# ssilverman16/particle_col_image_segmentation

Hardware: AMD Instinct MI355X
Metric: Mpixels/sec segmented (5-ch 1024x1024 TIFF), ROI mask IoU=1.0 (higher is better)
Workload: dtype f32 planes / u8 class maps / int32 labels / f64 ROI sums; 1 GPU; BASELINE config 2: batch of 64 frames 1024x1024x5 float32 per GPU, full kernel chain, inputs resident in HBM; frames_per_gpu=64, height=1024, width=1024, planes=5, parallelism=frames x1, launch=one hipGraph replay per step, 4 in flight, tie_fallback_frames_last_step=0, reference_nan_frames_rank0=0

## Files before the change

### particle_col_image_segmentation_amd/csrc/ccl.hip

```cpp
#include <type_traits>

#include "column_pass.h"
#include "tile_ops.h"

namespace pcseg {

constexpr int SCAN_PIX = 1024;

struct KeyEqU8 {
    const uint8_t *p;
    int W;
    int64_t n;
    __device__ __forceinline__ int operator()(int b, int r, int c) const { return p[b * n + rowoff(r, W) + c]; }
};
struct KeyNzU8 {
    const uint8_t *p;
    int W;
    int64_t n;
    __device__ __forceinline__ int operator()(int b, int r, int c) const { return p[b * n + rowoff(r, W) + c] != 0; }
};
struct KeyZeroU8 {
    const uint8_t *p;
    int W;
    int64_t n;
// ... 620 lines not shown
    if (ch == 0) u0 = u1l = u1r = 0;
    if (ch + 1 >= nch) d0 = d1l = d1r = 0;
    const unsigned cur1 = w0 | w1l | w1r, prev1 = u0 | u1l | u1r, next1 = d0 | d1l | d1r;
    unsigned acc = cur1 | w2l | w2r;
    acc |= (cur1 << 1) | (prev1 >> 31) | (cur1 >> 1) | (next1 << 31);
    acc |= (w0 << 2) | (u0 >> 30) | (w0 >> 2) | (d0 << 30);
    const int rows = min(32, H - ch * 32);
    acc &= col_valid(rows);
    out[((int64_t)b * nch + ch) * W + c] = acc;
}

constexpr int BR_TW = 64, BR_CH = 4, BR_ROWS = 32 * BR_CH;

__device__ __forceinline__ int bitrun_start(unsigned word, int p)
{
    const unsigned below = ~word & ((1u << p) - 1u);
    return below ? 32 - __clz(below) : 0;
}

template <typename Link>
__device__ __forceinline__ void bitrun_left_links(unsigned w, unsigned wl, Link &&link)
{
    unsigned rest = wl ? w : 0u;
    while (rest) {
        const int a = __ffs(rest) - 1;
        const unsigned from_a = w >> a;
        const int len = from_a == 0xFFFFFFFFu ? 32 : __ffs(~from_a) - 1;
        const int e = a + len - 1;
        rest = e >= 31 ? 0u : rest & ~((2u << e) - 1u);
        const int lo = max(a - 1, 0), hi = min(e + 1, 31);
        unsigned m = wl & (hi == 31 ? 0xFFFFFFFFu : ((2u << hi) - 1u)) & ~((1u << lo) - 1u);
        while (m) {
            const int p = __ffs(m) - 1;
            const int st = bitrun_start(wl, p);
            const unsigned from_p = wl >> p;
            const int run_len = from_p == 0xFFFFFFFFu ? 32 : __ffs(~from_p) - 1;
            const int en = p + run_len - 1;
            m = en >= 31 ? 0u : m & ~((2u << en) - 1u);
            link(a, st);
        }
    }
}

__global__ void __launch_bounds__(256) bitrun_tile_kernel(const unsigned *__restrict__ bits, int *__restrict__ parent, int H, int W,
                                                           int nch)
{
    __shared__ unsigned sw[BR_CH][BR_TW];
    __shared__ int lpar[BR_ROWS * BR_TW];
    const int col = threadIdx.x & (BR_TW - 1), q = threadIdx.x >> 6;
    const int c0 = blockIdx.x * BR_TW, ch0 = blockIdx.y * BR_CH, b = blockIdx.z;
    const int c = c0 + col, ch = ch0 + q;
    const unsigned w = (c < W && ch < nch) ? bits[((int64_t)b * nch + ch) * W + c] : 0u;
    sw[q][col] = w;
    for (unsigned heads = w & ~(w << 1); heads; heads &= heads - 1) {
        const int node = (q * 32 + (__ffs(heads) - 1)) * BR_TW + col;
        lpar[node] = node;
    }
    __syncthreads();
    if (w) {
        if (col > 0)
            bitrun_left_links(w, sw[q][col - 1], [&](int a, int st) {
                unite_lds(lpar, (q * 32 + a) * BR_TW + col, (q * 32 + st) * BR_TW + col - 1);
            });
        if ((w & 1u) && q > 0) {
            const int node = (q * 32) * BR_TW + col;
            const unsigned wu = sw[q - 1][col];
            if (wu >> 31) {
                unite_lds(lpar, node, ((q - 1) * 32 + bitrun_start(wu, 31)) * BR_TW + col);
            } else {
                if (col > 0 && (sw[q - 1][col - 1] >> 31))
                    unite_lds(lpar, node, ((q - 1) * 32 + bitrun_start(sw[q - 1][col - 1], 31)) * BR_TW + col - 1);
                if (col + 1 < BR_TW && (sw[q - 1][col + 1] >> 31))
                    unite_lds(lpar, node, ((q - 1) * 32 + bitrun_start(sw[q - 1][col + 1], 31)) * BR_TW + col + 1);
            }
        }
    }
    __syncthreads();
    int *par = parent + (int64_t)b * H * W;
    for (unsigned heads = w & ~(w << 1); heads; heads &= heads - 1) {
        const int node = (q * 32 + (__ffs(heads) - 1)) * BR_TW + col;
        const int root = find_lds(lpar, node);
        par[(ch0 * 32 + node / BR_TW) * W + c0 + node % BR_TW] = (ch0 * 32 + root / BR_TW) * W + c0 + root % BR_TW;
    }
}

__global__ void __launch_bounds__(256) bitrun_border_kernel(const unsigned *__restrict__ bits, int *__restrict__ parent, int H, int W,
                                                             int nch)
{
    const int c = blockIdx.x * 256 + threadIdx.x;
    const int ch = blockIdx.y, b = blockIdx.z;
    if (c >= W) return;
    const int col = c & (BR_TW - 1);
    const bool tile_left = col == 0 && c > 0, tile_top = (ch % BR_CH) == 0 && ch > 0;
    const bool edge_col = col == 0 || col == BR_TW - 1;
    if (!tile_left && !tile_top && !(edge_col && ch > 0)) return;
    const unsigned *wb = bits + (int64_t)b * nch * W;
    const int cl = c > 0 ? c - 1 : c, cr = c + 1 < W ? c + 1 : c, chu = ch > 0 ? ch - 1 : ch;
    const unsigned w = wb[rowoff(ch, W) + c], wl = wb[rowoff(ch, W) + cl];
    const unsigned wu = wb[rowoff(chu, W) + c], wul = wb[rowoff(chu, W) + cl], wur = wb[rowoff(chu, W) + cr];
    if (w == 0) return;
    int *par = parent + (int64_t)b * H * W;
    const int row0 = ch * 32;
    if (tile_left)
        bitrun_left_links(w, wl, [&](int a, int st) { unite_glb(par, (row0 + a) * W + c, (row0 + st) * W + c - 1); });
    if ((w & 1u) && ch > 0) {
        const int node = row0 * W + c;
        if (wu >> 31) {
            if (tile_top) unite_glb(par, node, (row0 - 32 + bitrun_start(wu, 31)) * W + c);
        } else {
            if (c > 0 && (tile_top || col == 0) && (wul >> 31)) unite_glb(par, node, (row0 - 32 + bitrun_start(wul, 31)) * W + c - 1);
            if (c + 1 < W && (tile_top || col == BR_TW - 1) && (wur >> 31))
                unite_glb(par, node, (row0 - 32 + bitrun_start(wur, 31)) * W + c + 1);
        }
    }
}

__global__ void __launch_bounds__(256) border_flag_kernel(const int *__restrict__ parent, uint8_t *__restrict__ flag, int H, int W)
{
    int t = blockIdx.x * blockDim.x + threadIdx.x;
    int r, c;
    if (t < W) { r = 0; c = t; }
    else if (t < 2 * W) { r = H - 1; c = t - W; }
    else if (t < 2 * W + H) { r = t - 2 * W; c = 0; }
    else if (t < 2 * W + 2 * H) { r = t - 2 * W - H; c = W - 1; }
    else return;
    int64_t fbase = (int64_t)blockIdx.y * H * W;
    int p = parent[fbase + rowoff(r, W) + c];
    if (p >= 0) flag[fbase + p] = 1;
}

__global__ void __launch_bounds__(256) fill_holes_out_kernel(const uint8_t *__restrict__ mask, const int *__restrict__ parent,
                                                              const uint8_t *__restrict__ flag, uint8_t *__restrict__ out, int64_t n)
{
    int64_t i = (int64_t)blockIdx.x * blockDim.x + threadIdx.x;
    if (i >= n) return;
    int64_t fbase = (int64_t)blockIdx.y * n;
    int p = parent[fbase + i];
    out[fbase + i] = (mask[fbase + i] != 0) || (p >= 0 && flag[fbase + p] == 0);
}

__global__ void __launch_bounds__(256) ccl_flatten_kernel(int *__restrict__ parent, int64_t n)
{
    int64_t i = (int64_t)blockIdx.x * blockDim.x + threadIdx.x;
    if (i >= n) return;
    int *par = parent + (int64_t)blockIdx.y * n;
    int p = par[i];
    if (p < 0 || !walk_ok((int)i, p)) return;
    const int x = walk_root(par, p);
    if (x != p) par[i] = x;
}

constexpr int LM_TW = CCL_TW, LM_TH = CCL_TH, LM_SW = LM_TW + 4, LM_SH = LM_TH + 4, LM_CW = LM_TW + 2, LM_CH = LM_TH + 2;

__global__ void __launch_bounds__(256) locmax_candidates_kernel(const int *__restrict__ img, unsigned long long *__restrict__ cbits,
                                                                 uint8_t *__restrict__ bad, int *__restrict__ nonconst,
                                                                 int *__restrict__ parent, int *__restrict__ markers, int H, int W)
{
    __shared__ int tile[LM_SH * LM_SW];
    __shared__ uint8_t cand[LM_CH * LM_CW];
    __shared__ int key[CCL_TILE];
    static_assert(LM_SH * LM_SW >= CCL_TILE, "the parents reuse the value tile");
    int *par = tile;
    const int OUTSIDE = (int)0x80000000;
    const TileIndex ti = xcd_tile_index();
    const int r0 = ti.y * LM_TH, c0 = ti.x * LM_TW;
    const int64_t fbase = (int64_t)ti.z * H * W;
    if ((W & 3) == 0 && c0 + LM_TW <= W && (((uintptr_t)img) & 15) == 0) {
        constexpr int QUADS = LM_SH * (LM_TW / 4), TRIPS = (QUADS + 255) / 256;
        int4 tq[TRIPS];
#pragma unroll
        for (int t = 0; t < TRIPS; ++t) {
            const int i = min((int)threadIdx.x + 256 * t, QUADS - 1);
            const int r = r0 + i / (LM_TW / 4) - 2;
            tq[t] = *reinterpret_cast<const int4 *>(img + fbase + rowoff(min(max(r, 0), H - 1), W) + c0 + 4 * (i % (LM_TW / 4)));
        }
        const int hl = min((int)threadIdx.x, LM_SH * 4 - 1);
        const int hr = r0 + (hl >> 2) - 2, hx = (hl & 3) < 2 ? (hl & 3) - 2 : LM_TW + (hl & 3) - 2, hc = c0 + hx;
        const int hv = img[fbase + rowoff(min(max(hr, 0), H - 1), W) + min(max(hc, 0), W - 1)];
#pragma unroll
        for (int t = 0; t < TRIPS; ++t) {
            const int i = (int)threadIdx.x + 256 * t;
            if (i < QUADS) {
                const int lr = i / (LM_TW / 4), r = r0 + lr - 2;
                const bool in = r >= 0 && r < H;
                int *dst = tile + lr * LM_SW + 2 + 4 * (i % (LM_TW / 4));
                dst[0] = in ? tq[t].x : OUTSIDE; dst[1] = in ? tq[t].y : OUTSIDE; dst[2] = in ? tq[t].z : OUTSIDE; dst[3] = in ? tq[t].w : OUTSIDE;
            }
        }
        if (threadIdx.x < LM_SH * 4) tile[(hl >> 2) * LM_SW + hx + 2] = (hr >= 0 && hr < H && hc >= 0 && hc < W) ? hv : OUTSIDE;
    } else {
        constexpr int TRIPS = (LM_SH * LM_SW + 255) / 256;
        int tv[TRIPS];
#pragma unroll
        for (int t = 0; t < TRIPS; ++t) {
            const int i = min((int)threadIdx.x + 256 * t, LM_SH * LM_SW - 1);
            const int r = r0 + i / LM_SW - 2, c = c0 + i % LM_SW - 2;
            tv[t] = img[fbase + rowoff(min(max(r, 0), H - 1), W) + min(max(c, 0), W - 1)];
        }
#pragma unroll
        for (int t = 0; t < TRIPS; ++t) {
            const int i = (int)threadIdx.x + 256 * t;
            const int r = r0 + i / LM_SW - 2, c = c0 + i % LM_SW - 2;
            if (i < LM_SH * LM_SW) tile[i] = (r >= 0 && r < H && c >= 0 && c < W) ? tv[t] : OUTSIDE;
        }
    }
    __syncthreads();
    const int first_value = img[fbase];
    bool any_differs = false;
    for (int t = threadIdx.x; t < LM_CH * LM_CW; t += 256) {
        const int lr = t / LM_CW, lc = t % LM_CW;
        const int r = r0 + lr - 1, c = c0 + lc - 1;
        const int i = (lr + 1) * LM_SW + lc + 1;
        const int v = tile[i];
        uint8_t state = 2;
        if (r >= 0 && r < H && c >= 0 && c < W) {
            const int *up = tile + i - LM_SW, *dn = tile + i + LM_SW;
            const int m = max(max(max(up[-1], up[0]), max(up[1], tile[i - 1])), max(max(tile[i + 1], dn[-1]), max(dn[0], dn[1])));
            state = m < v ? 1 : (m == v ? 3 : 0);
            any_differs = any_differs || v != first_value;
        }
        cand[t] = state;
    }
    __syncthreads();
    unsigned links = 0;
#pragma unroll
    for (int kk = 0; kk < LM_TH * LM_TW / 256; ++kk) {
        const int t = threadIdx.x + 256 * kk;
        const int lr = t / LM_TW, lc = t % LM_TW;
        const int r = r0 + lr, c = c0 + lc;
        int k = 0;
        if (r < H && c < W) {
            const int i = (lr + 2) * LM_SW + lc + 2, j = (lr + 1) * LM_CW + lc + 1;
            const int v = tile[i];
            const uint8_t st = cand[j];
            const bool is_cand = (st & 1) != 0;
            bool touches = false;
            if (st == 3) {
#pragma unroll
                for (int dr = -1; dr <= 1; ++dr)
#pragma unroll
                    for (int dc = -1; dc <= 1; ++dc) {
                        if (dr == 0 && dc == 0) continue;
                        const bool eq = tile[i + dr * LM_SW + dc] == v;
                        const uint8_t sn = cand[j + dr * LM_CW + dc];
                        touches = touches || (eq && sn == 0);
                        if ((dr < 0 || (dr == 0 && dc < 0)) && eq && (sn & 1) && lr + dr >= 0 && lc + dc >= 0 && lc + dc < LM_TW)
                            links |= 1u << (4 * kk + (dr == 0 ? 0 : dc + 2));
                    }
            }
            k = is_cand ? (v == 0 ? (int)0x80000000 : v) : 0;
            if (is_cand) bad[fbase + rowoff(r, W) + c] = touches ? 1 : 0;
            else if (markers) markers[fbase + rowoff(r, W) + c] = 0;
        }
        key[t] = k;
        const unsigned long long rowbits = __ballot(k != 0);
        if (lane_id() == 0 && r < H && rowbits) {
            const int64_t g = fbase + rowoff(r, W) + c0;
            const int sh = (int)(g & 63);
            atomicOr(cbits + (g >> 6), rowbits << sh);
            if (sh) atomicOr(cbits + (g >> 6) + 1, rowbits >> (64 - sh));
        }
    }
    if (__any(any_differs) && lane_id() == 0 && nonconst[ti.z] == 0) nonconst[ti.z] = 1;
    __syncthreads();
    for (int i = threadIdx.x; i < CCL_TILE; i += 256) par[i] = i;
    __syncthreads();
    if (links) {
#pragma unroll
        for (int kk = 0; kk < LM_TH * LM_TW / 256; ++kk) {
            const unsigned m = (links >> (4 * kk)) & 15u;
            if (!m) continue;
            const int i = threadIdx.x + 256 * kk;
            if (m & 1u) unite_lds_pair(par, i, i - 1);
            if (m & 2u) unite_lds_pair(par, i, i - CCL_TW - 1);
            if (m & 4u) unite_lds_pair(par, i, i - CCL_TW);
            if (m & 8u) unite_lds_pair(par, i, i - CCL_TW + 1);
        }
    }
    __syncthreads();
    for (int i = threadIdx.x; i < CCL_TILE; i += 256) {
        const int r = r0 + i / CCL_TW, c = c0 + i % CCL_TW;
        if (r >= H || c >= W || key[i] == 0) continue;
        const int root = find_lds(par, i);
        parent[fbase + rowoff(r, W) + c] = (r0 + root / CCL_TW) * W + c0 + root % CCL_TW;
    }
}

__global__ void __launch_bounds__(256) locmax_propagate_kernel(int *__restrict__ parent, uint8_t *bad,
                                                                const unsigned long long *__restrict__ cbits, int64_t n, int64_t total)
{
    const int64_t w = (int64_t)blockIdx.x * blockDim.x + threadIdx.x;
    if (w * 64 >= total) return;
    for (unsigned long long m = cbits[w]; m; m &= m - 1) {
        const int64_t g = w * 64 + (__ffsll((long long)m) - 1);
        const int64_t fbase = (g / n) * n;
        const int i = (int)(g - fbase);
        int *par = parent + fbase;
        const int p = par[i];
        if (!walk_ok(i, p)) continue;
        const int x = walk_root(par, p);
        if (x != p) par[i] = x;
        if (x != i && bad[g]) bad[fbase + x] = 1;
    }
}

__global__ void __launch_bounds__(256) locmax_out_kernel(const int *__restrict__ parent, const uint8_t *__restrict__ bad,
                                                          const int *__restrict__ nonconst, const unsigned long long *__restrict__ cbits,
                                                          uint8_t *__restrict__ is_max, int64_t n)
{
    int64_t i = (int64_t)blockIdx.x * blockDim.x + threadIdx.x;
    if (i >= n) return;
    const int64_t fbase = (int64_t)blockIdx.y * n;
    uint8_t v = 0;
    if (cand_bit(cbits, fbase + i)) v = bad[fbase + parent[fbase + i]] == 0 && nonconst[blockIdx.y] != 0;
    is_max[fbase + i] = v;
}

__device__ __forceinline__ unsigned long long cand_word(const unsigned long long *cbits, int b, int64_t i0, int64_t n)
{
    if (i0 >= n) return 0ull;
    const int64_t g0 = (int64_t)b * n + i0;
    const int sh = (int)(g0 & 63);
    unsigned long long w = cbits[g0 >> 6] >> sh;
    if (sh) w |= cbits[(g0 >> 6) + 1] << (64 - sh);
    if (n - i0 < 64) w &= (1ull << (n - i0)) - 1ull;
    return w;
}

static_assert(SCAN_PIX == 1024, "sixteen 64-bit words per count block");
template <typename Pred>
__global__ void __launch_bounds__(256) locmax_count_kernel(const int *__restrict__ parent, int *__restrict__ labels,
                                                            int *__restrict__ blockcount, const unsigned long long *__restrict__ cbits,
                                                            Pred pred, int64_t n, int nblk)
{
    const int b = blockIdx.y;
    const int *par = parent + (int64_t)b * n;
    const int64_t word = (int64_t)blockIdx.x * 256 + threadIdx.x;
    const int64_t i0 = word * 64;
    unsigned long long roots = 0;
    for (unsigned long long m = cand_word(cbits, b, i0, n); m; m &= m - 1) {
        const int j = __ffsll((long long)m) - 1;
        const int64_t i = i0 + j;
// ... 336 lines not shown
```

### particle_col_image_segmentation_amd/csrc/watershed.hip

```cpp
#include <algorithm>
#include <atomic>
#include <climits>
#include <mutex>
#include <type_traits>

#include "common.h"
#include "tile_rounds.h"

namespace pcseg {

constexpr int WS_T = 64;
constexpr unsigned WS_INF = 0xFFFFFFFFu;
constexpr int WS_CNT0 = 32, WS_CNT_STRIDE = 32, WS_CHANGED_INTS = WS_CNT0 + 16 * WS_CNT_STRIDE;

__device__ __forceinline__ unsigned ws_key(float f)
{
    if (f == 0.0f) f = 0.0f;
    unsigned u = __float_as_uint(f);
    u = (u & 0x80000000u) ? ~u : (u | 0x80000000u);
    return u == WS_INF ? WS_INF - 1 : u;
}

__global__ void __launch_bounds__(256) ws_init_kernel(const float *__restrict__ img, int64_t frame_stride,
                                                       const int *__restrict__ markers, const uint8_t *__restrict__ mask,
// ... 270 lines not shown
            if (oy >= 0 && oy < nxt.ny && ox >= 0 && ox < nxt.nx)
                mark_tile(dirty_out, list_out, count_out, ((int64_t)b * nxt.ny + oy) * nxt.nx + ox);
        }
    }
    __syncthreads();
    if (in.vec) {
#pragma unroll
        for (int t = 0; t < T * QW / NT; ++t) {
            const int idx = tid + NT * t, lr = idx / QW, q = idx % QW;
            const int r = r0 + lr, c = c0 + 4 * q;
            const uint2 *src = sLV + (lr + 1) * P + 1 + 4 * q;
            if (r >= 0 && r < H && c >= 0 && c < W)
                *reinterpret_cast<uint4 *>(L + fbase + rowoff(r, W) + c) = make_uint4(src[0].x, src[1].x, src[2].x, src[3].x);
        }
        return;
    }
    for (int i = tid; i < T * T; i += NT) {
        int lr = i / T, lc = i % T;
        int r = r0 + lr, c = c0 + lc;
        if (r >= 0 && r < H && c >= 0 && c < W) L[fbase + rowoff(r, W) + c] = sLV[(lr + 1) * P + lc + 1].x;
    }
}

__global__ void __launch_bounds__(RelaxGeom::THREADS) ws_relax_kernel(WsInputs in, const bool FIRST, unsigned *__restrict__ val,
                                                                         unsigned *__restrict__ L, uint8_t *__restrict__ dirty_in,
                                                                         uint8_t *__restrict__ dirty_out, int *__restrict__ any_changed,
                                                                         int H, int W, Tiling cur, Tiling nxt, int max_iter,
                                                                         int *__restrict__ list_out, int *__restrict__ count_out)
{
    extern __shared__ __attribute__((aligned(16))) uint2 relax_lds[];
    const TileIndex t = xcd_tile_index();
    ws_relax_tile(relax_lds + RelaxGeom::PAD, in, FIRST, val, L, dirty_in, dirty_out, any_changed, H, W, cur, nxt, max_iter, t.x, t.y,
                     t.z, list_out, count_out);
}

constexpr int WS_LIST_FROM = 4, WS_LIST_GRID = 1024;

__global__ void __launch_bounds__(RelaxGeom::THREADS) ws_relax_list_kernel(WsInputs in, unsigned *__restrict__ val, unsigned *__restrict__ L,
                                                                           uint8_t *__restrict__ dirty_in, uint8_t *__restrict__ dirty_out,
                                                                           int *__restrict__ any_changed, int H, int W, Tiling cur,
                                                                           Tiling nxt, int max_iter, TileList tiles,
                                                                           int *__restrict__ list_out, int *__restrict__ count_out)
{
    extern __shared__ __attribute__((aligned(16))) uint2 relax_lds[];
    for_tiles(tiles, [&](const int b, const int tx, const int ty) {
        ws_relax_tile(relax_lds + RelaxGeom::PAD, in, false, val, L, dirty_in, dirty_out, any_changed, H, W, cur, nxt, max_iter, tx, ty, b,
                      list_out, count_out);
        __syncthreads();
    });
}

__global__ void __launch_bounds__(RelaxGeom::THREADS) ws_relax_tail_kernel(WsInputs in, unsigned *__restrict__ val, unsigned *__restrict__ L,
                                                                           uint8_t *__restrict__ dirtyA, uint8_t *__restrict__ dirtyB,
                                                                           int *__restrict__ any_changed, int *__restrict__ not_converged,
                                                                           int *__restrict__ exact_flags, int H, int W, Tiling t0,
                                                                           Tiling t1, int first_round, int max_rounds)
{
    extern __shared__ __attribute__((aligned(16))) uint2 relax_lds[];
    const int b = blockIdx.x;
    const int rounds = tail_rounds<RelaxGeom::THREADS>(
        b, dirtyA, dirtyB, first_round, max_rounds, t0, t1, [](const int) { return true; },
        [&](const Tiling &cur, const Tiling &nxt, const int tx, const int ty, uint8_t *din, uint8_t *dout) {
            ws_relax_tile(relax_lds + RelaxGeom::PAD, in, false, val, L, din, dout, any_changed, H, W, cur, nxt, 100000, tx, ty, b);
        });
    if (rounds < 0 && threadIdx.x == 0) { *not_converged = 1; exact_flags[b] = 1; }
}

__device__ __forceinline__ bool ws_active(const uint8_t *active, int b, int r, int c, int tilesX, int tilesY)
{
    return active == nullptr || active[((int64_t)b * tilesY + r / WS_T) * tilesX + c / WS_T] != 0;
}

__global__ void __launch_bounds__(256) ws_list_tiles_kernel(const int *__restrict__ frame_list, const uint8_t *__restrict__ active, int ntpf,
                                                             int *__restrict__ tile_list)
{
    ws_for_frames(frame_list, blockIdx.x, gridDim.x, [&](const int b) {
        for (int t = threadIdx.x; t < ntpf; t += 256)
            if (active[(int64_t)b * ntpf + t]) tile_list[atomicAdd(&tile_list[-1], 1)] = b * ntpf + t;
    });
}

constexpr int UF_TW = 64, UF_TH = 32, UF_SW = UF_TW + 2, UF_SH = UF_TH + 2;
constexpr int UF_LNS = UF_TW * UF_TH;
constexpr int UF_NS = 1 << 30;

__device__ __forceinline__ int vfind_lds(int *par, int v)
{
    int p;
    while ((p = ld_lds(par + (v & (UF_LNS - 1)))) != v) {
        const int g = ld_lds(par + (p & (UF_LNS - 1)));
        if (g != p) st_lds(par + (v & (UF_LNS - 1)), g);
        v = g;
    }
    return v;
}
__device__ __forceinline__ void vunite_lds(int *par, int a, int b)
{
    for (;;) {
        a = vfind_lds(par, a);
        b = vfind_lds(par, b);
        if (a == b) return;
        if (a < b) { int t = a; a = b; b = t; }
        int old = atomicMin(&par[a & (UF_LNS - 1)], b);
        if (old == a) return;
        a = old;
    }
}
__device__ __forceinline__ bool vwalk_ok(int x, int p, int n) { return (unsigned)p <= (unsigned)x && (p & (UF_NS - 1)) < n; }

__device__ __forceinline__ void vunite_glb(int *par, int p, int q, int n, int *corrupt)
{
    int a = ld_agent(par + p), b = ld_agent(par + q);
    bool ok = a >= 0 && b >= 0 && (a & (UF_NS - 1)) < n && (b & (UF_NS - 1)) < n;
    while (ok) {
        for (;;) {
            if (a == b) return;
            const int pa = ld_agent(par + (a & (UF_NS - 1))), pb = ld_agent(par + (b & (UF_NS - 1)));
            if (pa == a && pb == b) break;
            if (!vwalk_ok(a, pa, n) || !vwalk_ok(b, pb, n)) { ok = false; break; }
            const int ga = ld_agent(par + (pa & (UF_NS - 1))), gb = ld_agent(par + (pb & (UF_NS - 1)));
            if (!vwalk_ok(pa, ga, n) || !vwalk_ok(pb, gb, n)) { ok = false; break; }
            if (pa != a) {
                if (ga != pa) __hip_atomic_store(par + (a & (UF_NS - 1)), ga, __ATOMIC_RELAXED, __HIP_MEMORY_SCOPE_AGENT);
                a = ga;
            }
            if (pb != b) {
                if (gb != pb) __hip_atomic_store(par + (b & (UF_NS - 1)), gb, __ATOMIC_RELAXED, __HIP_MEMORY_SCOPE_AGENT);
                b = gb;
            }
        }
        if (!ok) break;
        if (a == b) return;
        if (a < b) { int t = a; a = b; b = t; }
        int old = atomicMin(par + (a & (UF_NS - 1)), b);
        if (old == a) return;
        if (!vwalk_ok(a, old, n)) break;
        a = old;
    }
    walk_corrupt(corrupt);
}
__device__ __forceinline__ int vwalk_root(const int *par, int x, int n, bool &bad)
{
    int q;
    while ((q = par[x & (UF_NS - 1)]) != x) {
        if (!vwalk_ok(x, q, n)) {
            bad = true;
            break;
        }
        x = q;
    }
    return x;
}

template <typename KeyT>
__device__ __forceinline__ void ws_uf_tile_frame(KeyT *sK, int *par, uint8_t *sM, const int b, const int tile_x, const int tile_y,
                                                 const KeyT *__restrict__ K,
                                                 const int *__restrict__ F, const uint8_t *__restrict__ active,
                                                 int *__restrict__ parent, uint8_t *__restrict__ minmask, uint8_t *__restrict__ bad,
                                                 int H, int W, int tilesX, int tilesY)
{
    const KeyT KINF = ~(KeyT)0;
    const int r0 = tile_y * UF_TH, c0 = tile_x * UF_TW;
    if (!ws_active(active, b, r0, c0, tilesX, tilesY)) return;
    const int64_t fbase = (int64_t)b * H * W;
    if (sizeof(KeyT) == 4 && (W & 3) == 0 && c0 + UF_TW <= W && (((uintptr_t)K) & 15) == 0) {
        constexpr int QUADS = UF_SH * (UF_TW / 4), TRIPS = (QUADS + 255) / 256;
        uint4 kq[TRIPS];
#pragma unroll
        for (int t = 0; t < TRIPS; ++t) {
            const int i = min((int)threadIdx.x + 256 * t, QUADS - 1);
            const int r = r0 + i / (UF_TW / 4) - 1;
            kq[t] = *reinterpret_cast<const uint4 *>(K + fbase + rowoff(min(max(r, 0), H - 1), W) + c0 + 4 * (i % (UF_TW / 4)));
        }
        const int hl = min((int)threadIdx.x, UF_SH * 2 - 1);
        const int hr = r0 + (hl >> 1) - 1, hx = (hl & 1) ? UF_TW : -1, hc = c0 + hx;
        const KeyT hv = K[fbase + rowoff(min(max(hr, 0), H - 1), W) + min(max(hc, 0), W - 1)];
#pragma unroll
        for (int t = 0; t < TRIPS; ++t) {
            const int i = (int)threadIdx.x + 256 * t;
            if (i < QUADS) {
                const int lr = i / (UF_TW / 4), r = r0 + lr - 1;
                const bool in = r >= 0 && r < H;
                KeyT *dst = sK + lr * UF_SW + 1 + 4 * (i % (UF_TW / 4));
                dst[0] = in ? (KeyT)kq[t].x : KINF; dst[1] = in ? (KeyT)kq[t].y : KINF;
                dst[2] = in ? (KeyT)kq[t].z : KINF; dst[3] = in ? (KeyT)kq[t].w : KINF;
            }
        }
        if (threadIdx.x < UF_SH * 2) sK[(hl >> 1) * UF_SW + hx + 1] = (hr >= 0 && hr < H && hc >= 0 && hc < W) ? hv : KINF;
    } else {
        constexpr int TRIPS = (UF_SH * UF_SW + 255) / 256;
        KeyT kv[TRIPS];
#pragma unroll
        for (int t = 0; t < TRIPS; ++t) {
            const int i = min((int)threadIdx.x + 256 * t, UF_SH * UF_SW - 1);
            const int r = r0 + i / UF_SW - 1, c = c0 + i % UF_SW - 1;
            kv[t] = K[fbase + rowoff(min(max(r, 0), H - 1), W) + min(max(c, 0), W - 1)];
        }
#pragma unroll
        for (int t = 0; t < TRIPS; ++t) {
            const int i = (int)threadIdx.x + 256 * t;
            const int r = r0 + i / UF_SW - 1, c = c0 + i % UF_SW - 1;
            if (i < UF_SH * UF_SW) sK[i] = (r >= 0 && r < H && c >= 0 && c < W) ? kv[t] : KINF;
        }
    }
    __syncthreads();
    int self[UF_LNS / 256];
    int fv[UF_LNS / 256];
#pragma unroll
    for (int k = 0; k < UF_LNS / 256; ++k) {
        const int t = threadIdx.x + k * 256;
        fv[k] = F[fbase + rowoff(min(r0 + t / UF_TW, H - 1), W) + min(c0 + t % UF_TW, W - 1)];
    }
#pragma unroll
    for (int k = 0; k < UF_LNS / 256; ++k) {
        const int t = threadIdx.x + k * 256;
        const int lr = t / UF_TW, lc = t % UF_TW;
        const int r = r0 + lr, c = c0 + lc;
        const int i = (lr + 1) * UF_SW + lc + 1;
        int v = -1;
        if ((unsigned)(sK[i] >> (8 * sizeof(KeyT) - 32)) != WS_INF)
            v = fv[k] != 0 ? t : t + UF_LNS;
        uint8_t m8 = 0;
        if (v >= UF_LNS) {
            const KeyT ku = sK[i - UF_SW], kl = sK[i - 1], kr = sK[i + 1], kd = sK[i + UF_SW];
            const KeyT m = min(min(ku, kd), min(kl, kr));
            if (m != KINF) m8 = (ku == m ? 1 : 0) | (kl == m ? 2 : 0) | (kr == m ? 4 : 0) | (kd == m ? 8 : 0);
        }
        self[k] = v;
        sM[t] = m8;
        if (r < H && c < W) {
            minmask[fbase + rowoff(r, W) + c] = m8;
            if (fv[k] != 0) bad[fbase + rowoff(r, W) + c] = 0;
        }
    }
    __syncthreads();
#pragma unroll
    for (int k = 0; k < UF_LNS / 256; ++k) {
        const int t = threadIdx.x + k * 256;
        const int lc = t % UF_TW;
        const bool joins_left = lc > 0 && ((sM[t] & 2) || (sM[t - 1] & 4));
        const unsigned long long heads = __ballot(!joins_left);
        const unsigned long long seeds = __ballot(self[k] >= 0 && self[k] < UF_LNS);
        const unsigned long long upto = heads & (lc == 63 ? ~0ull : ((2ull << lc) - 1ull));
        const int start = 63 - __clzll((long long)upto);
        const unsigned long long later = lc == 63 ? 0ull : (heads >> (lc + 1));
        const int end = later ? lc + (__ffsll((long long)later) - 1) : 63;
        const unsigned long long run = (end == 63 ? ~0ull : ((2ull << end) - 1ull)) & ~((1ull << start) - 1ull);
        const unsigned long long run_seeds = seeds & run;
        int root = -1;
        if (self[k] >= 0) {
            if (run_seeds) root = (t - lc) + (__ffsll((long long)run_seeds) - 1);
            else root = (t - lc) + start + UF_LNS;
        }
        par[t] = root;
    }
    __syncthreads();
#pragma unroll
    for (int k = 0; k < UF_LNS / 256; ++k) {
        const int t = threadIdx.x + k * 256;
        const int lr = t / UF_TW, lc = t % UF_TW;
        if (lr == 0 || self[k] < 0) continue;
        const uint8_t m = sM[t], mu = sM[t - UF_TW];
        if (!((m & 1) || (mu & 8))) continue;
        if (lc > 0) {
            const uint8_t ml = sM[t - 1], mul = sM[t - UF_TW - 1];
            const bool same_run = (m & 2) || (ml & 4), same_run_up = (mu & 2) || (mul & 4), left_vertical = (ml & 1) || (mul & 8);
            if (same_run && same_run_up && left_vertical) continue;
        }
        vunite_lds(par, par[t], par[t - UF_TW]);
    }
    __syncthreads();
    for (int t = threadIdx.x; t < UF_TH * UF_TW; t += 256) {
        const int r = r0 + t / UF_TW, c = c0 + t % UF_TW;
        if (r >= H || c >= W) continue;
        int v = -1;
        if (par[t] >= 0) {
            const int root = vfind_lds(par, par[t]);
            const int lt = root & (UF_LNS - 1);
            v = ((r0 + lt / UF_TW) * W + c0 + lt % UF_TW) | (root >= UF_LNS ? UF_NS : 0);
        }
        parent[fbase + rowoff(r, W) + c] = v;
    }
}

template <typename KeyT, bool LIST>
__global__ void __launch_bounds__(256) ws_uf_tile_kernel(TileList tiles, const KeyT *__restrict__ K, const int *__restrict__ F,
                                                          const uint8_t *__restrict__ active, int *__restrict__ parent,
                                                          uint8_t *__restrict__ minmask, uint8_t *__restrict__ bad, int H, int W,
                                                          int tilesX, int tilesY)
{
    __shared__ KeyT sK[UF_SH * UF_SW];
    __shared__ int par[UF_TH * UF_TW];
    __shared__ uint8_t sM[UF_LNS];
    if constexpr (!LIST) {
        const TileIndex t = xcd_tile_index();
        ws_uf_tile_frame<KeyT>(sK, par, sM, t.z, t.x, t.y, K, F, active, parent, minmask, bad, H, W, tilesX, tilesY);
    } else {
        for_tiles(tiles, [&](const int b, const int tx, const int ty) {
            for (int half = 0; half < WS_T / UF_TH; ++half) {
                if ((ty * (WS_T / UF_TH) + half) * UF_TH < H)
                    ws_uf_tile_frame<KeyT>(sK, par, sM, b, tx, ty * (WS_T / UF_TH) + half, K, F, active, parent, minmask, bad, H, W, tilesX,
                                           tilesY);
                __syncthreads();
            }
        });
    }
}

__global__ void __launch_bounds__(256, 8) ws_uf_border_kernel(const int *__restrict__ frame_list, const uint8_t *__restrict__ minmask, const uint8_t *__restrict__ active,
                                                            int *__restrict__ parent, int H, int W, int tilesX, int tilesY,
                                                            int *__restrict__ exact_flags)
{
    const int n_top_rows = (H - 1) / UF_TH, n_edges = (W - 1) / UF_TW;
    int i = blockIdx.x * 256 + threadIdx.x;
    int r, c;
    if (i < n_top_rows * W) {
        r = (i / W + 1) * UF_TH;
        c = i % W;
    } else {
        i -= n_top_rows * W;
        if (i >= n_edges * H) return;
        r = i % H;
        if ((r % UF_TH) == 0 && r > 0) return;
        c = (i / H + 1) * UF_TW;
    }
    ws_for_frames(frame_list, blockIdx.y, gridDim.y, [&](const int b) {
    if (!ws_active(active, b, r, c, tilesX, tilesY)) return;
    const bool top = (r % UF_TH) == 0 && r > 0;
    const bool left = (c % UF_TW) == 0 && c > 0;
    if (!top && !left) return;
    const int64_t fbase = (int64_t)b * H * W;
    int *par = parent + fbase;
    const int p = r * W + c;
    const uint8_t *mm = minmask + fbase;
    const int up = r > 0 ? W : 0, lf = c > 0 ? 1 : 0;
    const uint8_t mp = mm[p], mu = mm[p - up], ml = mm[p - lf], mul = mm[p - up - lf];
    if (top && ws_active(active, b, r - 1, c, tilesX, tilesY)) {
        if ((mp & 1) || (mu & 8)) {
            bool implied = false;
            if (!left && c > 0) implied = ((mp & 2) || (ml & 4)) && ((mu & 2) || (mul & 4)) && ((ml & 1) || (mul & 8));
            if (!implied) vunite_glb(par, p, p - W, H * W, exact_flags + b);
        }
    }
    if (left && ws_active(active, b, r, c - 1, tilesX, tilesY)) {
        if ((mp & 2) || (ml & 4)) {
            bool implied = false;
            if (!top && r > 0) implied = ((mp & 1) || (mu & 8)) && ((ml & 1) || (mul & 8)) && ((mu & 2) || (mul & 4));
            if (!implied) vunite_glb(par, p, p - 1, H * W, exact_flags + b);
        }
    }
    });
}

enum { UF_OPTIMISTIC = 0, UF_REPAIR = 1, UF_DETECT = 2, UF_ASSIGN = 3 };

template <int MODE>
__device__ __forceinline__ void ws_uf_label_pixel(const int b, const int64_t i, const int *__restrict__ parent, int *__restrict__ F,
                                                  const uint8_t *__restrict__ active, uint8_t *__restrict__ bad,
                                                  const int *__restrict__ markers, const uint8_t *__restrict__ mask,
                                                  int *__restrict__ tie_flags, uint8_t *__restrict__ mark_active, int64_t n, int W,
                                                  int tilesX, int tilesY, int *__restrict__ exact_flags, uint8_t *__restrict__ in_bad,
                                                  uint8_t *__restrict__ mark_dirty)
{
    const int r = (int)(i / W), c = (int)(i % W);
    if (i >= n || !ws_active(active, b, r, c, tilesX, tilesY)) return;
    const int64_t fbase = (int64_t)b * n, g = fbase + i;
    if (MODE == UF_REPAIR && in_bad) in_bad[g] = 0;
    int x = parent[g];
    if (x < 0) return;
    const int *par = parent + fbase;
    bool broken = (x & (UF_NS - 1)) >= (int)n;
    if (!broken) x = vwalk_root(par, x, (int)n, broken);
    if (broken) {
        exact_flags[b] = 1;
        return;
    }
    if (x >= UF_NS) return;
    const int64_t groot = fbase + x;
    if (MODE == UF_REPAIR) {
        if (bad[groot]) {
            F[g] = mask[g] ? markers[g] : 0;
            if (mark_active) mark_active[((int64_t)b * tilesY + r / WS_T) * tilesX + c / WS_T] = 1;
            if (mark_dirty) mark_dirty[((int64_t)b * tilesY + r / WS_T) * tilesX + c / WS_T] = 1;
            if (in_bad) in_bad[g] = 1;
        }
        return;
    }
    const int f = F[g];
    if (MODE == UF_ASSIGN) {
        if (f == 0 && !bad[groot]) F[g] = F[groot];
        return;
    }
    const int lab = F[groot];
    if (f == 0) {
        if (MODE == UF_OPTIMISTIC) F[g] = lab;
    } else if (f != lab) {
        bad[groot] = 1;
        if (tie_flags[b] == 0) tie_flags[b] = 1;
    }
}

template <int MODE>
__global__ void __launch_bounds__(256) ws_uf_label_kernel(const int *__restrict__ frame_list, const int *__restrict__ parent, int *__restrict__ F,
                                                           const uint8_t *__restrict__ active, uint8_t *__restrict__ bad,
                                                           const int *__restrict__ markers, const uint8_t *__restrict__ mask,
                                                           int *__restrict__ tie_flags, uint8_t *__restrict__ mark_active, int64_t n,
                                                           int W, int tilesX, int tilesY, int *__restrict__ exact_flags,
                                                           uint8_t *__restrict__ in_bad = nullptr, uint8_t *__restrict__ mark_dirty = nullptr)
{
    const int64_t i = (int64_t)blockIdx.x * blockDim.x + threadIdx.x;
    ws_for_frames(frame_list, blockIdx.y, gridDim.y, [&](const int b) {
        ws_uf_label_pixel<MODE>(b, i, parent, F, active, bad, markers, mask, tie_flags, mark_active, n, W, tilesX, tilesY, exact_flags,
                                in_bad, mark_dirty);
    });
}

template <int MODE>
__global__ void __launch_bounds__(256) ws_uf_label_tiles_kernel(TileList tiles, const int *__restrict__ parent, int *__restrict__ F,
                                                                 const uint8_t *__restrict__ active, uint8_t *__restrict__ bad,
                                                                 const int *__restrict__ markers, const uint8_t *__restrict__ mask,
                                                                 int *__restrict__ tie_flags, int H, int W, int tilesX, int tilesY,
                                                                 int *__restrict__ exact_flags)
{
    for_tiles(tiles, [&](const int b, const int tx, const int ty) {
        ws_for_tile_pixels(tx, ty, H, W, [&](const int r, const int c) {
            ws_uf_label_pixel<MODE>(b, (int64_t)r * W + c, parent, F, active, bad, markers, mask, tie_flags, nullptr, (int64_t)H * W, W,
                                    tilesX, tilesY, exact_flags, nullptr, nullptr);
        });
    });
}

constexpr int LABEL4_Q = 3;

template <int NCH>
__device__ __forceinline__ void label4_chains(const int *par, const int *F, int64_t fbase, int n, int (&root)[NCH], int (&lab)[NCH], bool &bad)
{
    const int n1 = n - 1;
    int cut = 0;
    bool more = true;
    while (more) {
        int nx[NCH];
#pragma unroll
        for (int q = 0; q < NCH; ++q) {
            const unsigned px = (unsigned)(root[q] & (INT_MIN | (UF_NS - 1)));
            nx[q] = px <= (unsigned)n1 ? par[min(px, (unsigned)n1)] : -1;
        }
// ... 987 lines not shown
```

Baseline: 17550 Mpixels/s.

## Add wave-ballot row pass for watershed UF tile and quad-vectorized locmax candidates

```diff
diff --git a/particle_col_image_segmentation_amd/csrc/ccl.hip b/particle_col_image_segmentation_amd/csrc/ccl.hip
--- a/particle_col_image_segmentation_amd/csrc/ccl.hip
+++ b/particle_col_image_segmentation_amd/csrc/ccl.hip
@@ -796,12 +796,142 @@
 
 constexpr int LM_TW = CCL_TW, LM_TH = CCL_TH, LM_SW = LM_TW + 4, LM_SH = LM_TH + 4, LM_CW = LM_TW + 2, LM_CH = LM_TH + 2;
 
+constexpr int LM_CP = 72;
+__device__ __forceinline__ uint8_t locmax_state(const int *tile, int i, int v)
+{
+    const int *up = tile + i - LM_SW, *dn = tile + i + LM_SW;
+    const int m = max(max(max(up[-1], up[0]), max(up[1], tile[i - 1])), max(max(tile[i + 1], dn[-1]), max(dn[0], dn[1])));
+    return m < v ? 1 : (m == v ? 3 : 0);
+}
+__device__ __forceinline__ void locmax_tile_quads(int *tile, uint8_t *cand, int *key, const int64_t fbase, const int r0, const int c0,
+                                                  const int frame, const int *__restrict__ img, unsigned long long *__restrict__ cbits,
+                                                  uint8_t *__restrict__ bad, int *__restrict__ nonconst, int *__restrict__ parent,
+                                                  int *__restrict__ markers, int H, int W)
+{
+    const int tid = threadIdx.x, lr = 2 * (tid >> 4), lc = 4 * (tid & 15);
+    unsigned *rowbits = reinterpret_cast<unsigned *>(key);
+    if (tid < 2 * LM_TH) rowbits[tid] = 0;
+    const int first_value = img[fbase];
+    bool any_differs = false;
+    unsigned st4[2];
+    {
+        int h[4][4], e[2][4], v[2][4];
+#pragma unroll
+        for (int rr = 0; rr < 4; ++rr) {
+            const int4 *p = reinterpret_cast<const int4 *>(tile + (lr + 1 + rr) * LM_SW + lc);
+            const int4 a0 = p[0], a1 = p[1];
+            const int a[8] = {a0.x, a0.y, a0.z, a0.w, a1.x, a1.y, a1.z, a1.w};
+#pragma unroll
+            for (int c = 0; c < 4; ++c) {
+                h[rr][c] = max(max(a[1 + c], a[2 + c]), a[3 + c]);
+                if (rr == 1 || rr == 2) { e[rr - 1][c] = max(a[1 + c], a[3 + c]); v[rr - 1][c] = a[2 + c]; }
+            }
+        }
+#pragma unroll
+        for (int o = 0; o < 2; ++o) {
+            const bool in = r0 + lr + o < H;
+            unsigned w = 0;
+#pragma unroll
+            for (int c = 0; c < 4; ++c) {
+                const int m = max(max(h[o][c], e[o][c]), h[o + 2][c]);
+                const unsigned st = !in ? 2u : (m < v[o][c] ? 1u : (m == v[o][c] ? 3u : 0u));
+                w |= st << (8 * c);
+                any_differs = any_differs || (in && v[o][c] != first_value);
+            }
+            st4[o] = w;
+            *reinterpret_cast<unsigned *>(cand + (lr + o + 1) * LM_CP + 4 + lc) = w;
+        }
+    }
+    if (tid < 2 * LM_CW + 2 * LM_TH) {
+        int rl, cl;
+        if (tid < 2 * LM_CW) { rl = tid < LM_CW ? -1 : LM_TH; cl = (tid < LM_CW ? tid : tid - LM_CW) - 1; }
+        else { rl = (tid - 2 * LM_CW) >> 1; cl = (tid & 1) ? LM_TW : -1; }
+        const int r = r0 + rl, c = c0 + cl, i = (rl + 2) * LM_SW + cl + 2;
+        cand[(rl + 1) * LM_CP + 4 + cl] = (r >= 0 && r < H && c >= 0 && c < W) ? locmax_state(tile, i, tile[i]) : 2;
+    }
+    __syncthreads();
+    unsigned links = 0;
+#pragma unroll
+    for (int o = 0; o < 2; ++o) {
+        const int r = r0 + lr + o;
+        if (r >= H) continue;
+        const int64_t g = fbase + rowoff(r, W) + c0 + lc;
+        if ((st4[o] & 0x01010101u) == 0) {
+            if (markers) *reinterpret_cast<int4 *>(markers + g) = make_int4(0, 0, 0, 0);
+            continue;
+        }
+        unsigned nib = 0;
+        for (int c = 0; c < 4; ++c) {
+            const unsigned st = (st4[o] >> (8 * c)) & 0xffu;
+            if (!(st & 1u)) {
+                if (markers) markers[g + c] = 0;
+                continue;
+            }
+            bool touches = false;
+            if (st == 3) {
+                const int i = (lr + o + 2) * LM_SW + lc + c + 2, j = (lr + o + 1) * LM_CP + 4 + lc + c;
+                const int v = tile[i];
+#pragma unroll
+                for (int dr = -1; dr <= 1; ++dr)
+#pragma unroll
+                    for (int dc = -1; dc <= 1; ++dc) {
+                        if (dr == 0 && dc == 0) continue;
+                        const bool eq = tile[i + dr * LM_SW + dc] == v;
+                        const uint8_t sn = cand[j + dr * LM_CP + dc];
+                        touches = touches || (eq && sn == 0);
+                        if ((dr < 0 || (dr == 0 && dc < 0)) && eq && (sn & 1) && lr + o + dr >= 0 && lc + c + dc >= 0 && lc + c + dc < LM_TW)
+                            links |= 1u << (4 * (4 * o + c) + (dr == 0 ? 0 : dc + 2));
+                    }
+            }
+            bad[g + c] = touches ? 1 : 0;
+            nib |= 1u << c;
+        }
+        atomicOr(&rowbits[2 * (lr + o) + (lc >> 5)], nib << (lc & 31));
+    }
+    if (__any(any_differs) && lane_id() == 0 && nonconst[frame] == 0) nonconst[frame] = 1;
+    __syncthreads();
+    int *par = tile;
+    if (tid < LM_TH && r0 + tid < H) {
+        const unsigned long long rb = (unsigned long long)rowbits[2 * tid] | ((unsigned long long)rowbits[2 * tid + 1] << 32);
+        if (rb) {
+            const int64_t g = fbase + rowoff(r0 + tid, W) + c0;
+            const int sh = (int)(g & 63);
+            atomicOr(cbits + (g >> 6), rb << sh);
+            if (sh) atomicOr(cbits + (g >> 6) + 1, rb >> (64 - sh));
+        }
+    }
+    const unsigned cb0 = st4[0] & 0x01010101u, cb1 = (r0 + lr + 1 < H) ? st4[1] & 0x01010101u : 0u;
+    const bool any_cand = (r0 + lr < H) && (cb0 | cb1);
+    if (any_cand)
+        for (int kk = 0; kk < 8; ++kk)
+            if (((kk < 4 ? cb0 : cb1) >> (8 * (kk & 3))) & 1u) { const int i = (lr + (kk >> 2)) * CCL_TW + lc + (kk & 3); par[i] = i; }
+    __syncthreads();
+    if (links)
+        for (int kk = 0; kk < 8; ++kk) {
+            const unsigned m = (links >> (4 * kk)) & 15u;
+            if (!m) continue;
+            const int i = (lr + (kk >> 2)) * CCL_TW + lc + (kk & 3);
+            if (m & 1u) unite_lds_pair(par, i, i - 1);
+            if (m & 2u) unite_lds_pair(par, i, i - CCL_TW - 1);
+            if (m & 4u) unite_lds_pair(par, i, i - CCL_TW);
+            if (m & 8u) unite_lds_pair(par, i, i - CCL_TW + 1);
+        }
+    __syncthreads();
+    if (any_cand)
+        for (int kk = 0; kk < 8; ++kk)
+            if (((kk < 4 ? cb0 : cb1) >> (8 * (kk & 3))) & 1u) {
+                const int i = (lr + (kk >> 2)) * CCL_TW + lc + (kk & 3);
+                const int root = find_lds(par, i);
+                parent[fbase + rowoff(r0 + i / CCL_TW, W) + c0 + i % CCL_TW] = (r0 + root / CCL_TW) * W + c0 + root % CCL_TW;
+            }
+}
+
 __global__ void __launch_bounds__(256) locmax_candidates_kernel(const int *__restrict__ img, unsigned long long *__restrict__ cbits,
                                                                  uint8_t *__restrict__ bad, int *__restrict__ nonconst,
                                                                  int *__restrict__ parent, int *__restrict__ markers, int H, int W)
 {
-    __shared__ int tile[LM_SH * LM_SW];
-    __shared__ uint8_t cand[LM_CH * LM_CW];
+    __shared__ __attribute__((aligned(16))) int tile[LM_SH * LM_SW];
+    __shared__ __attribute__((aligned(4))) uint8_t cand[LM_CH * LM_CP];
     __shared__ int key[CCL_TILE];
     static_assert(LM_SH * LM_SW >= CCL_TILE, "the parents reuse the value tile");
     int *par = tile;
@@ -832,6 +962,11 @@
             }
         }
         if (threadIdx.x < LM_SH * 4) tile[(hl >> 2) * LM_SW + hx + 2] = (hr >= 0 && hr < H && hc >= 0 && hc < W) ? hv : OUTSIDE;
+        if ((((uintptr_t)markers) & 15) == 0) {
+            __syncthreads();
+            locmax_tile_quads(tile, cand, key, fbase, r0, c0, ti.z, img, cbits, bad, nonconst, parent, markers, H, W);
+            return;
+        }
     } else {
         constexpr int TRIPS = (LM_SH * LM_SW + 255) / 256;
         int tv[TRIPS];
diff --git a/particle_col_image_segmentation_amd/csrc/watershed.hip b/particle_col_image_segmentation_amd/csrc/watershed.hip
--- a/particle_col_image_segmentation_amd/csrc/watershed.hip
+++ b/particle_col_image_segmentation_amd/csrc/watershed.hip
@@ -446,6 +446,102 @@
     return x;
 }
 
+__device__ __forceinline__ void vunite_roots_lds(int *par, int a, int b)
+{
+    if (a == b) return;
+    if (a < b) { int t = a; a = b; b = t; }
+    const int old = atomicMin(&par[a & (UF_LNS - 1)], b);
+    if (old != a) vunite_lds(par, old, b);
+}
+
+__device__ __forceinline__ bool lane_bit(unsigned long long m) { return __builtin_amdgcn_inverse_ballot_w64(m); }
+__device__ __forceinline__ unsigned long long ballot64(bool p) { return __builtin_amdgcn_ballot_w64(p); }
+__device__ __forceinline__ unsigned scan_high(unsigned x) { unsigned r; asm("v_ffbh_u32 %0, %1" : "=v"(r) : "v"(x)); return r; }
+__device__ __forceinline__ unsigned scan_low(unsigned x) { unsigned r; asm("v_ffbl_b32 %0, %1" : "=v"(r) : "v"(x)); return r; }
+__device__ __forceinline__ unsigned scan_low64(unsigned long long x) { return min(scan_low((unsigned)x), scan_low((unsigned)(x >> 32)) | 32u); }
+__device__ __forceinline__ unsigned long long uniform64(unsigned long long x)
+{
+    return (unsigned long long)(unsigned)__builtin_amdgcn_readfirstlane((unsigned)x) |
+           ((unsigned long long)(unsigned)__builtin_amdgcn_readfirstlane((unsigned)(x >> 32)) << 32);
+}
+
+__device__ __forceinline__ void ws_uf_tile_rows(const unsigned *sK, int *par, unsigned long long *sX, const int64_t fbase, const int r0,
+                                                const int c0, const int *__restrict__ F, int *__restrict__ parent,
+                                                uint8_t *__restrict__ minmask, uint8_t *__restrict__ bad, int H, int W)
+{
+    typedef unsigned long long u64;
+    constexpr int ROWS = UF_TH / 4;
+    static_assert(UF_TW == WAVE && ROWS * 4 == UF_TH && UF_LNS == 1 << 11, "a lane per column, four waves");
+    const unsigned lane = lane_id();
+    const int w = __builtin_amdgcn_readfirstlane(threadIdx.x >> 6);
+    const int lr0 = w * ROWS;
+    const int64_t base = fbase + rowoff(r0 + lr0, W) + c0;
+    uint8_t *const mm_row0 = minmask + base, *const bad_row0 = bad + base;
+    int *const parent_row0 = parent + base;
+    int fv[ROWS];
+#pragma unroll
+    for (int k = 0; k < ROWS; ++k) fv[k] = (F + (fbase + rowoff(min(r0 + lr0 + k, H - 1), W) + c0))[lane];
+    const u64 le_mask = lane == 63 ? ~0ull : ((2ull << lane) - 1ull);
+    u64 need[ROWS];
+    u64 Jp = 0, Dp = 0, U0 = 0, J0 = 0, R0 = 0;
+    unsigned ku = sK[lr0 * UF_SW + lane + 1], kc = sK[(lr0 + 1) * UF_SW + lane + 1];
+#pragma unroll
+    for (int k = 0; k < ROWS; ++k) {
+        const int lr = lr0 + k, i = (lr + 1) * UF_SW + lane + 1;
+        const unsigned kd = sK[i + UF_SW], kl = sK[i - 1], kr = sK[i + 1];
+        const unsigned m = min(min(ku, kd), min(kl, kr));
+        const u64 R = ballot64(kc != WS_INF);
+        const u64 Z = ballot64(fv[k] == 0);
+        const u64 S = R & ~Z;
+        const u64 live = R & Z & ballot64(m != WS_INF);
+        const u64 U = live & ballot64(ku == m), L = live & ballot64(kl == m), Rt = live & ballot64(kr == m), D = live & ballot64(kd == m);
+        const u64 J = (L | (Rt << 1)) & ~1ull;
+        const unsigned off = lane + k * W;
+        if (r0 + lr < H) {
+            mm_row0[off] = (uint8_t)((lane_bit(U) ? 1 : 0) | (lane_bit(L) ? 2 : 0) | (lane_bit(Rt) ? 4 : 0) | (lane_bit(D) ? 8 : 0));
+            if (lane_bit(~Z)) bad_row0[off] = 0;
+        }
+        const u64 V = U | Dp;
+        need[k] = V & R & ~(J & Jp & (V << 1));
+        if (k == 0) { U0 = U; J0 = J; R0 = R; }
+        const u64 heads = ~J;
+        const u64 below = heads & le_mask;
+        const int start = 63 ^ (int)min(scan_high((unsigned)(below >> 32)), scan_high((unsigned)below) | 32u);
+        const u64 s1 = S >> start, h1 = ((heads >> 1) | (1ull << 63)) >> start;
+        const unsigned fs = scan_low64(s1), nh = scan_low64(h1);
+        const int root = (lr * UF_TW + start) + (fs <= nh ? (int)fs : UF_LNS);
+        par[lr * UF_TW + lane] = lane_bit(R) ? root : -1;
+        ku = kc; kc = kd; Jp = J; Dp = D;
+    }
+    if (w + 1 < 4 && lane == 0) { sX[2 * w] = Jp; sX[2 * w + 1] = Dp; }
+    __syncthreads();
+    need[0] = 0;
+    if (w > 0) {
+        const u64 Ju = uniform64(sX[2 * w - 2]), V = U0 | uniform64(sX[2 * w - 1]);
+        need[0] = V & R0 & ~(J0 & Ju & (V << 1));
+    }
+#pragma unroll
+    for (int k = 0; k < ROWS; ++k)
+        if (lane_bit(need[k])) {
+            const int t = (lr0 + k) * UF_TW + lane;
+            vunite_roots_lds(par, par[t], par[t - UF_TW]);
+        }
+    __syncthreads();
+    const int px0 = r0 * W + c0;
+#pragma unroll
+    for (int k = 0; k < ROWS; ++k) {
+        if (r0 + lr0 + k >= H) break;
+        const int p = par[(lr0 + k) * UF_TW + lane];
+        int v = -1;
+        if (p >= 0) {
+            const int root = vfind_lds(par, p);
+            const int lt = root & (UF_LNS - 1);
+            v = (px0 + __mul24(lt >> 6, W - UF_TW) + lt) | ((root & UF_LNS) << 19);
+        }
+        parent_row0[lane + k * W] = v;
+    }
+}
+
 template <typename KeyT>
 __device__ __forceinline__ void ws_uf_tile_frame(KeyT *sK, int *par, uint8_t *sM, const int b, const int tile_x, const int tile_y,
                                                  const KeyT *__restrict__ K,
@@ -481,6 +577,11 @@
             }
         }
         if (threadIdx.x < UF_SH * 2) sK[(hl >> 1) * UF_SW + hx + 1] = (hr >= 0 && hr < H && hc >= 0 && hc < W) ? hv : KINF;
+        if constexpr (sizeof(KeyT) == 4) {
+            __syncthreads();
+            ws_uf_tile_rows((const unsigned *)sK, par, reinterpret_cast<unsigned long long *>(sM), fbase, r0, c0, F, parent, minmask, bad, H, W);
+            return;
+        }
     } else {
         constexpr int TRIPS = (UF_SH * UF_SW + 255) / 256;
         KeyT kv[TRIPS];
@@ -585,7 +686,7 @@
 {
     __shared__ KeyT sK[UF_SH * UF_SW];
     __shared__ int par[UF_TH * UF_TW];
-    __shared__ uint8_t sM[UF_LNS];
+    __shared__ __attribute__((aligned(8))) uint8_t sM[UF_LNS];
     if constexpr (!LIST) {
         const TileIndex t = xcd_tile_index();
         ws_uf_tile_frame<KeyT>(sK, par, sM, t.z, t.x, t.y, K, F, active, parent, minmask, bad, H, W, tilesX, tilesY);
diff --git a/profiles/tile_pass_valu/count_insts.py b/profiles/tile_pass_valu/count_insts.py
--- /dev/null
+++ b/profiles/tile_pass_valu/count_insts.py
@@ -0,0 +1,65 @@
+import re
+import sys
+
+
+def classify(op):
+    if op.startswith("v_"):
+        return "valu"
+    if op.startswith("ds_"):
+        return "lds"
+    if op.startswith(("global_", "flat_", "buffer_")):
+        return "vmem"
+    if op.startswith("s_waitcnt") or op.startswith("s_nop"):
+        return "wait"
+    if op.startswith("s_load") or op.startswith("s_buffer_load"):
+        return "smem"
+    if op.startswith("s_"):
+        return "salu"
+    return "other"
+
+
+def main():
+    path, sub = sys.argv[1], sys.argv[2]
+    lines = open(path).read().splitlines()
+    start = next(i for i, l in enumerate(lines) if re.match(r"^_Z\w*:", l) and sub in l)
+    end = next(i for i in range(start, len(lines)) if lines[i].strip().startswith(".end_amdhsa_kernel"))
+    blocks, cur = [], ["entry", {}]
+    res = {}
+    for l in lines[start + 1:end]:
+        s = l.strip()
+        if s.startswith(".amdhsa_"):
+            k, _, v = s.partition(" ")
+            if k in (".amdhsa_next_free_vgpr", ".amdhsa_next_free_sgpr", ".amdhsa_group_segment_fixed_size",
+                     ".amdhsa_private_segment_fixed_size", ".amdhsa_accum_offset"):
+                res[k[8:]] = v.strip()
+            continue
+        m = re.match(r"^(\.LBB\w+):", s)
+        if m:
+            blocks.append(cur)
+            cur = [m.group(1), {}]
+            continue
+        if not s or s.startswith((";", ".")):
+            continue
+        c = classify(s.split()[0])
+        cur[1][c] = cur[1].get(c, 0) + 1
+    blocks.append(cur)
+    tot = {}
+    for _, d in blocks:
+        for k, v in d.items():
+            tot[k] = tot.get(k, 0) + v
+    print(lines[start].rstrip(":"))
+    print("static:", " ".join("%s=%d" % kv for kv in sorted(tot.items())))
+    print("resources:", " ".join("%s=%s" % kv for kv in sorted(res.items())))
+    for l in lines[end:end + 400]:
+        if re.search(r"; (NumVgprs|NumSgprs|ScratchSize|Occupancy|LDSByteSize|NumAgprs)", l):
+            print(l.strip())
+        if l.strip().startswith(".section") or re.match(r"^_Z\w*:", l):
+            break
+    if "--blocks" in sys.argv:
+        for name, d in blocks:
+            if d:
+                print("%-14s %s" % (name, " ".join("%s=%d" % kv for kv in sorted(d.items()))))
+
+
+if __name__ == "__main__":
+    main()
diff --git a/profiles/tile_pass_valu/kernel_times.py b/profiles/tile_pass_valu/kernel_times.py
--- /dev/null
+++ b/profiles/tile_pass_valu/kernel_times.py
@@ -0,0 +1,27 @@
+import json
+import os
+import sys
+
+import torch
+
+sys.path.insert(0, os.path.join(os.path.dirname(os.path.abspath(__file__)), "..", ".."))
+import bench
+from particle_col_image_segmentation_amd import _lib, synth
+from particle_col_image_segmentation_amd.pipeline import FramePipeline
+
+STEPS = 4
+lib = _lib.load()
+dev = torch.device("cuda")
+stack = synth.gen_batch_torch(10_000, 64, 1024, 1024, dev)
+solo = FramePipeline(dict(synth.CELL_TYPES_5), overlap=False)
+for _ in range(2):
+    solo.run(stack)
+torch.cuda.synchronize()
+kernels, _, _ = bench._timing_pass(lib, lambda: [solo.run(stack) for _ in range(STEPS)], torch.cuda.synchronize)
+out = {"lib": os.environ.get("PCSEG_LIB", "branch"), "steps": STEPS,
+       "serial_us_per_step": round(1e3 * sum(ms for _, ms in kernels.values()) / STEPS, 1)}
+for name, (calls, ms) in kernels.items():
+    short = name.lstrip("(").split("(")[0].strip()
+    if "locmax_candidates_kernel" in name or ("ws_uf_tile_kernel" in name and "false" in name):
+        out[short] = {"launches_per_step": calls / STEPS, "us_per_step": round(1e3 * ms / STEPS, 1)}
+print(json.dumps(out))
diff --git a/profiles/tile_pass_valu/pmc_steps.py b/profiles/tile_pass_valu/pmc_steps.py
--- /dev/null
+++ b/profiles/tile_pass_valu/pmc_steps.py
@@ -0,0 +1,14 @@
+import os
+import sys
+
+import torch
+
+sys.path.insert(0, os.path.join(os.path.dirname(os.path.abspath(__file__)), "..", ".."))
+from particle_col_image_segmentation_amd import synth
+from particle_col_image_segmentation_amd.pipeline import FramePipeline
+
+stack = synth.gen_batch_torch(10_000, 64, 1024, 1024, torch.device("cuda"))
+solo = FramePipeline(dict(synth.CELL_TYPES_5), overlap=False)
+for _ in range(2):
+    solo.run(stack)
+torch.cuda.synchronize()
diff --git a/profiles/tile_pass_valu/pmc_summary.py b/profiles/tile_pass_valu/pmc_summary.py
--- /dev/null
+++ b/profiles/tile_pass_valu/pmc_summary.py
@@ -0,0 +1,25 @@
+import csv
+import glob
+import json
+import sys
+
+PIXELS = 64 * 1024 * 1024
+acc = {}
+for path in glob.glob(sys.argv[1] + "/**/*counter_collection.csv", recursive=True):
+    with open(path, newline="") as f:
+        for row in csv.DictReader(f):
+            name = row["Kernel_Name"]
+            if "locmax_candidates_kernel" in name:
+                k = "locmax_candidates_kernel"
+            elif "ws_uf_tile_kernel" in name and ("false" in name or "Lb0" in name) and ("unsigned int" in name or "IjL" in name):
+                k = "ws_uf_tile_kernel<unsigned, false>"
+            else:
+                continue
+            d = acc.setdefault(k, {}).setdefault(row["Counter_Name"], [0.0, 0])
+            d[0] += float(row["Counter_Value"])
+            d[1] += 1
+out = {}
+for k, counters in acc.items():
+    out[k] = {c: {"launches": n, "per_launch": v / n, "wave64_instructions_per_pixel": round(v / n * 64 / PIXELS, 1)}
+              for c, (v, n) in counters.items()}
+print(json.dumps(out))
```

Result: slower. 16900 Mpixels/s (-3.7%).
